# ishine/minimax-speech

Measured on NVIDIA B200. Metric: audio-sec synthesized/sec (24 kHz), higher is better.
Workload: dtype bf16

## Files before the change

minimax-speech_b200/csrc/c_api.cu:

```cuda
#include <atomic>
#include <cstdarg>
#include <mutex>
#include <vector>

#include "dac_enc_engine.h"
#include "dac_engine.h"
#include "engine_common.h"
#include "f32_path.h"
#include "flow_engine.h"
#include "front_engine.h"
#include "profiler.h"
#include "s3_engine.h"

namespace ls {

std::atomic<long long> g_launch_count{0};
long long* g_debug_buffer = nullptr;
bool pdl_enabled() {
  static const bool on = [] {
    const char* e = getenv("LS_NO_PDL");
    return !(e && e[0] == '1');
  }();
  return on;
}
long long g_debug_bytes = 0;
int conv_halo_mode() {
  static const int mode = [] {
    const char* e = getenv("LS_CONV_HALO");
    return e && e[0] >= '0' && e[0] <= '2' ? e[0] - '0' : 2;
  }();
  return mode;
}
bool conv_halo_enabled() { return conv_halo_mode() != 0; }
bool conv_fuse_res_enabled() {
  static const bool on = [] {
    const char* e = getenv("LS_CONV_FUSE_RES");
    return !(e && e[0] == '0');
  }();
  return on;
}
bool conv_dual_enabled() {
  static const bool on = [] {
    const char* e = getenv("LS_CONV_DUAL");
    return !(e && e[0] == '0');
  }();
  return on;
}
bool conv_tma_out_enabled() {
  static const bool on = [] {
    const char* e = getenv("LS_CONV_TMA_OUT");
    return !(e && e[0] == '0');
// ... 666 lines not shown
```

minimax-speech_b200/csrc/conv_gemm.cu:

```cuda
#include <cstdio>
#include <string>
#include <unordered_map>

#include "kernels.h"
#include "profiler.h"
#include "ptx.cuh"

namespace ls {
namespace {

constexpr int kBlockM = 128;
constexpr int kBlockK = 64;
constexpr int kEpiWarps = 16;
constexpr int kEpiThreads = kEpiWarps * 32;
#ifndef CONV_PRODUCER_WARPS
#define CONV_PRODUCER_WARPS 3
#endif
constexpr int kProducerWarps = CONV_PRODUCER_WARPS;
constexpr int kWeightProducers = kProducerWarps - 1;
static_assert(kProducerWarps >= 2, "need one activation and at least one weight producer");
constexpr int kMmaWarp = kProducerWarps;
constexpr int kFirstEpiWarp = kProducerWarps + 1;
constexpr int kThreads = kFirstEpiWarp * 32 + kEpiThreads;
constexpr int kMaxStages = 16;
// ... 234 lines not shown
  fence_proxy_async_smem();
  __syncwarp();
  if (lane == 0) {
    tma_store_3d(map, kF32 ? stg : stg + kOff, n, t_base, b);
    bulk_commit();
  }
}

template <int kKind, int kOff = kStageB16Off>
__device__ __forceinline__ void store_chunk_tma_p(bool one_pending, uint8_t* stg, int lane, const CUtensorMap* map, int n,
                                                  int t_base, int b, bool row_valid, const float (&v)[16]) {
  if (one_pending) store_chunk_tma<kKind, 1, kOff>(stg, lane, map, n, t_base, b, row_valid, v);
  else store_chunk_tma<kKind, 0, kOff>(stg, lane, map, n, t_base, b, row_valid, v);
}

template <int kAct, int kOut0, int kOut1, int kAdd, int kTemb>
__global__ void __launch_bounds__(kThreads, 1)
conv_gemm_kernel(const __grid_constant__ CUtensorMap mapA0, const __grid_constant__ CUtensorMap mapA1,
                 const __grid_constant__ CUtensorMap mapW, const __grid_constant__ CUtensorMap mapOut0,
                 const __grid_constant__ CUtensorMap mapOut1, const __grid_constant__ ConvGemmParams p,
                 const int tmem_cols, const int acc_stride) {
  const int act = kAct >= 0 ? kAct : p.act;
  const int out0_dtype = kOut0 >= 0 ? kOut0 : p.out0_dtype;
  const int out1_mode = kOut1 >= 0 ? kOut1 : p.out1_mode;
  const int add_dtype = kAdd >= 0 ? kAdd : (p.addend_dtype == ADD_GEMM ? (int)ADD_GEMM : p.addend ? p.addend_dtype : (int)OUT_NONE);
  const bool has_temb = kTemb >= 0 ? kTemb != 0 : p.temb != nullptr;
  extern __shared__ uint8_t smem_raw[];
  uint8_t* smem = reinterpret_cast<uint8_t*>((reinterpret_cast<uintptr_t>(smem_raw) + 1023) & ~uintptr_t(1023));
  const int a_bytes = ls_conv_a_stage_bytes(p.a_box_rows);
  const int b_bytes = p.block_n * kBlockK * 2;
  uint8_t* smem_a = smem;
  uint8_t* smem_b = smem + (size_t)p.a_stages * a_bytes;
  uint64_t* bars = reinterpret_cast<uint64_t*>(smem_b + (size_t)p.b_stages * b_bytes);
  uint64_t* a_full = bars;
  uint64_t* a_empty = bars + kMaxStages;
  uint64_t* b_full = bars + 2 * kMaxStages;
  uint64_t* b_empty = bars + 3 * kMaxStages;
  uint64_t* tfull = bars + 4 * kMaxStages;
  uint64_t* tempty = tfull + 2;
  uint32_t* tmem_slot = reinterpret_cast<uint32_t*>(tempty + 2);
  float2* red_base = reinterpret_cast<float2*>(bars + 128);
  uint8_t* stg_base = reinterpret_cast<uint8_t*>(red_base) + p.red_bytes;
  float* svec = reinterpret_cast<float*>(stg_base + kEpiWarps * kStageBytesPerWarp);

  const int warp = threadIdx.x >> 5;
  const int lane = threadIdx.x & 31;
  const int m_tiles = (p.M + kBlockM - 1) / kBlockM;
  const int n_tiles = p.N / p.block_n;
  const int total_tiles = p.B * m_tiles * n_tiles;
  const bool halo = p.halo_mode != 0;
  long long* tl = p.timeline ? p.timeline + (size_t)blockIdx.x * 64 : nullptr;
#define TL(i)                    \
  do {                           \
    if (tl) tl[(i)] = clock64(); \
  } while (0)
// ... 24 lines not shown
      const int tap = r / p.kb_per_tap, kb = r - tap * p.kb_per_tap;
      tma_prefetch_l2_2d(&mapW, kb * kBlockK, tap * p.N + nt * p.block_n);
    }
    for (int j = blockIdx.x; j < p.res_kb; j += gridDim.x) tma_prefetch_l2_2d(&p.res_w, j * kBlockK, 0);
  }
  if (warp == kMmaWarp && lane == 0) {
    for (int i = 0; i < kMaxStages; ++i) {
      mbar_init(&a_full[i], 1);
      mbar_init(&a_empty[i], 1);
      mbar_init(&b_full[i], 1);
      mbar_init(&b_empty[i], (p.dual && !p.b_resident) ? 2 : 1);
    }
    for (int i = 0; i < 2; ++i) {
      mbar_init(&tfull[i], 1);
      mbar_init(&tempty[i], kEpiThreads);
    }
    fence_barrier_init();
  }
  if (warp == 0) {
    __syncwarp();
    tmem_alloc(tmem_slot, (uint32_t)tmem_cols);
    tmem_relinquish();
  }
  {
    auto stage_vec = [&](int off, const float* src, int n) {
      if (off >= 0)
        for (int i = threadIdx.x; i < n; i += kThreads) svec[off + i] = __ldg(src + i);
    };
    stage_vec(p.sv_bias, p.bias, p.chan_mod);
    stage_vec(p.sv_p1a, p.p1_a, p.chan_mod);
    stage_vec(p.sv_p1b, p.p1_b, p.chan_mod);
    stage_vec(p.sv_lng, p.ln_g, p.N);
    stage_vec(p.sv_lnb, p.ln_b, p.N);
  }
  pdl_launch_dependents();
  tc_fence_before();
  __syncthreads();
  tc_fence_after();
  const uint32_t tmem_base = *tmem_slot;
  if (threadIdx.x == 0) TL(1);
  pdl_wait();
  if (threadIdx.x == 0) TL(2);

  auto next_tile = [&](int& cur) -> int {
    while (cur < total_tiles) {
      const int t = cur;
      cur += (int)gridDim.x;
      if (!tile_skipped(p, decode_tile(t, m_tiles, n_tiles))) return t;
    }
    return -1;
  };
  if (p.dual && warp < 2) {
    if (lane == 0) {
      const int depth = p.a_stages >> 1;
      const uint32_t a_tx = (uint32_t)p.a_box_rows * 128u;
      int cur = blockIdx.x, pair = 0, bs = 0;
      uint32_t bph = 0;
      int cnt[2] = {0, 0};
      for (;; ++pair) {
        int t[2];
        t[0] = next_tile(cur);
        if (t[0] < 0) break;
        t[1] = next_tile(cur);
        if (warp == 1 && (!p.b_resident || pair == 0)) {
          for (int kb = 0; kb < p.kb_per_tap; ++kb)
// ... 65 lines not shown
            if (!p.b_resident) {
              umma_commit(&b_empty[bl]);
              if (lone) umma_commit(&b_empty[bl]);
            }
            if (++bl == p.b_stages) bl = 0, bphl ^= 1;
          }
          umma_commit(&a_empty[st]);
        }
        __syncwarp();
        for (int tap = 0; tap < p.taps; ++tap)
          if (++bs == p.b_stages) bs = 0, bph ^= 1;
        ++cnt;
      }
      if (elect_one()) umma_commit(&tfull[m]);
      __syncwarp();
      acc_phase ^= 1;
    }
  } else if (warp < kProducerWarps) {
    if (lane == 0) {
      int as = 0, bs = 0;
      uint32_t aph = 0, bph = 0;
      int b_seq = 0, p_tile = 0;
      int a_seq = 0;
#if CONV_DETAIL_TL == 2
      int dn = 0;
#endif
      const bool a_share = p.b_resident && p.a_stages >= kProducerWarps;
      const uint32_t a_tx = (uint32_t)p.a_box_rows * 128u;
      for (int tile = blockIdx.x; tile < total_tiles; tile += gridDim.x) {
        const TileCoord tc = decode_tile(tile, m_tiles, n_tiles);
// ... 55 lines not shown
            }
            if (++b_seq == kWeightProducers) b_seq = 0;
            if (++bs == p.b_stages) bs = 0, bph ^= 1;
          }
        }
      }
    }
  } else if (warp == kMmaWarp) {
    {
      const uint32_t tmem_u = __shfl_sync(0xffffffffu, tmem_base, 0);
      const uint32_t idesc = make_idesc_bf16(kBlockM, p.block_n, false, false);
      int as = 0, bs = 0;
      uint32_t aph = 0, bph = 0;
      int acc = 0;
      uint32_t acc_phase = 0;
      int n_it = 0, n_tile = 0;
      for (int tile = blockIdx.x; tile < total_tiles; tile += gridDim.x) {
        const TileCoord tc = decode_tile(tile, m_tiles, n_tiles);
        if (__shfl_sync(0xffffffffu, (int)tile_skipped(p, tc), 0)) continue;
        mbar_wait(&tempty[acc], acc_phase ^ 1);
        tc_fence_after();
        const uint32_t d_tmem = tmem_u + (uint32_t)(acc * acc_stride);
        if (halo && p.b_resident && n_tile > 0) {
          for (int kb = 0; kb < p.kb_per_tap; ++kb) {
            mbar_wait(&a_full[as], aph);
            tc_fence_after();
            int nk = kBlockK / 16;
            if (p.k_true > 0 && p.kb_split == p.kb_per_tap) nk = min(nk, (p.k_true - kb * kBlockK + 15) >> 4);
            const uint32_t a_addr = smem_u32(smem_a + (size_t)as * a_bytes);
            const uint32_t b_addr = smem_u32(smem_b) + (uint32_t)(kb * p.taps) * (uint32_t)b_bytes;
// ... 83 lines not shown
#pragma unroll
              for (int k = 0; k < kBlockK / 16; ++k)
                if (k < nk) umma_bf16(d_tmem, adesc + 2 * k, bdesc + 2 * k, idesc, (kb | tap | k) != 0 ? 1u : 0u);
              if (!p.b_resident) umma_commit(&b_empty[bs]);
              if (a_done) umma_commit(&a_empty[as]);
            }
            __syncwarp();
            if (++bs == p.b_stages) bs = 0, bph ^= 1;
            if (a_done) {
              if (++as == p.a_stages) as = 0, aph ^= 1;
            }
          }
        }
        if (elect_one()) umma_commit(&tfull[acc]);
        __syncwarp();
        if (p.res_kb > 0) {
          const uint32_t d2 = tmem_u + (uint32_t)((acc ^ 1) * acc_stride);
          for (int kb2 = 0; kb2 < p.res_kb; ++kb2) {
            mbar_wait(&a_full[as], aph);
            mbar_wait(&b_full[bs], bph);
            tc_fence_after();
            const int nk2 = min(kBlockK / 16, (p.res_k_true - kb2 * kBlockK + 15) >> 4);
            const uint64_t adesc = make_smem_desc_sw128(smem_u32(smem_a + (size_t)as * a_bytes));
            const uint64_t bdesc = make_smem_desc_sw128(smem_u32(smem_b + (size_t)bs * b_bytes));
            if (elect_one()) {
#pragma unroll
              for (int k = 0; k < kBlockK / 16; ++k)
                if (k < nk2) umma_bf16(d2, adesc + 2 * k, bdesc + 2 * k, idesc, (kb2 | k) != 0 ? 1u : 0u);
              umma_commit(&b_empty[bs]);
              umma_commit(&a_empty[as]);
            }
            __syncwarp();
            if (++as == p.a_stages) as = 0, aph ^= 1;
            if (++bs == p.b_stages) bs = 0, bph ^= 1;
          }
          if (elect_one()) umma_commit(&tfull[acc ^ 1]);
          __syncwarp();
        }
        if (tl && lane == 0 && n_it <= p.taps * p.kb_per_tap) tl[32] = clock64();
        if (tl && lane == 0 && n_tile < 8) tl[24 + n_tile] = clock64();
        ++n_tile;
        acc ^= 1;
        if (acc == 0) acc_phase ^= 1;
      }
    }
  } else {
    const int q = warp & 3;
    const int g = (warp - kFirstEpiWarp) >> 2;
    const int row = q * 32 + lane;
    const int n_chunks = p.block_n >> 4;
    uint8_t* stg = stg_base + (warp - kFirstEpiWarp) * kStageBytesPerWarp;
    int acc = 0;
    uint32_t acc_phase = 0;
    uint32_t parity = 0;
    int e_tile = 0;
    for (int tile = blockIdx.x; tile < total_tiles; tile += gridDim.x) {
      const TileCoord tc = decode_tile(tile, m_tiles, n_tiles);
      const int t = tc.mt * kBlockM + row;
      const int n0 = tc.nt * p.block_n;
// ... 57 lines not shown
        const int nxt = tile + (int)gridDim.x;
        if (nxt < total_tiles) {
          const TileCoord nc = decode_tile(nxt, m_tiles, n_tiles);
          const int esz = add_dtype == OUT_F32 ? 4 : 2;
          const int lines = (p.block_n * esz + 127) >> 7;
          const uint8_t* nb = reinterpret_cast<const uint8_t*>(p.addend) + (long long)nc.b * p.out_bstride * esz;
          for (int i = threadIdx.x - kFirstEpiWarp * 32; i < kBlockM * lines; i += kEpiThreads) {
            const int rr = i / lines, ln = i - rr * lines;
            const long long tt = (long long)nc.mt * kBlockM + rr;
            const long long f = tt * p.out_ld + p.out_shift + nc.nt * p.block_n;
            if (tt < p.M && f >= 0 && f + p.block_n <= p.out_alloc)
              asm volatile("prefetch.global.L2 [%0];" ::"l"(nb + f * esz + ln * 128));
          }
        }
      }
      mbar_wait(&tfull[acc], acc_phase);
      tc_fence_after();
      long long* tle = (threadIdx.x == kFirstEpiWarp * 32 && tile == (int)blockIdx.x) ? tl : nullptr;
      if (tle) tle[40] = clock64();
      const uint32_t taddr = tmem_base + ((uint32_t)(q * 32) << 16) + (uint32_t)(acc * acc_stride);
      auto load_x = [&](int c, float (&x)[16]) {
        tmem_ld16(taddr + (uint32_t)(c * 16), reinterpret_cast<uint32_t(&)[16]>(x));
        tmem_ld_wait();
        if (p.bias) {
          const int ch0 = (n0 + c * 16) % p.chan_mod;
          const float4* bp = reinterpret_cast<const float4*>(p.sv_bias >= 0 ? svec + p.sv_bias + ch0 : p.bias + ch0);
#pragma unroll
          for (int g4 = 0; g4 < 4; ++g4) {
            const float4 bv = bp[g4];
            x[4 * g4] += bv.x, x[4 * g4 + 1] += bv.y, x[4 * g4 + 2] += bv.z, x[4 * g4 + 3] += bv.w;
          }
        }
        if (act == ACT_LRELU || act == ACT_LRELU_TANH) {
#pragma unroll
          for (int i = 0; i < 16; ++i) x[i] = x[i] > 0.f ? x[i] : 0.1f * x[i];
// ... 217 lines not shown
  __syncthreads();
  if (threadIdx.x == 0) TL(44);
  if (warp == 0) {
    tc_fence_after();
    tmem_dealloc(tmem_base, (uint32_t)tmem_cols);
  }
#undef TL
}

int pow2_at_least(int x, int lo) {
  int v = lo;
  while (v < x) v <<= 1;
  return v;
}

template <int kAct, int kOut0, int kOut1, int kAdd, int kTemb>
cudaError_t launch_instance(int grid, size_t smem, cudaStream_t stream, const CUtensorMap& mapA0, const CUtensorMap& mapA1,
                            const CUtensorMap& mapW, const CUtensorMap& mapO0, const CUtensorMap& mapO1,
                            const ConvGemmParams& pp, int tmem_cols, int acc_stride) {
  auto* kernel = conv_gemm_kernel<kAct, kOut0, kOut1, kAdd, kTemb>;
  static std::atomic<unsigned long long> optin{0};
  if (cudaError_t e = smem_optin_once(optin, reinterpret_cast<const void*>(kernel), 227 * 1024); e != cudaSuccess) return e;
  return launch_pdl(kernel, dim3(grid), dim3(kThreads), smem, stream, 1, mapA0, mapA1, mapW, mapO0, mapO1, pp, tmem_cols,
                    acc_stride);
}

}

cudaError_t LS_FN(launch_conv_gemm)(const CUtensorMap& mapA0, const CUtensorMap& mapA1, const CUtensorMap& mapW,
                                    const ConvGemmParams& p, int num_sms, cudaStream_t stream) {
#if !LS_HALF_FP16
  if (p.fp16) return launch_conv_gemm_fp16(mapA0, mapA1, mapW, p, num_sms, stream);
#endif
  if (p.block_n % 16 || p.block_n < 16 || p.block_n > 256 || p.N % p.block_n || p.chan_mod % 16) return cudaErrorInvalidValue;
  if ((p.act == ACT_LN_MISH || p.out1_mode == OUT1_LN) && p.block_n != p.N) return cudaErrorInvalidValue;
  if (p.out1_mode == OUT1_LN && p.out0_dtype != OUT_F32) return cudaErrorInvalidValue;
  if (p.out1_mode != OUT1_NONE && p.out1 == nullptr) return cudaErrorInvalidValue;
  if (p.addend_dtype == ADD_GEMM) {
    const long long tiles = (long long)p.B * ((p.M + kBlockM - 1) / kBlockM);
    if (p.res_kb <= 0 || p.res_bias == nullptr || p.N != p.block_n || tiles > num_sms) return cudaErrorInvalidValue;
  } else if (p.res_kb != 0) {
    return cudaErrorInvalidValue;
  }
  ConvGemmParams pp = p;
  pp.timeline = (g_debug_buffer && g_debug_bytes >= 148 * 64 * 8) ? g_debug_buffer : nullptr;
  pp.a_box_rows = p.halo_mode ? conv_halo_box_rows(p.taps, p.dil) : kBlockM;
  if (pp.a_box_rows > 256) return cudaErrorInvalidValue;
  const int a_bytes = ls_conv_a_stage_bytes(pp.a_box_rows);
  const int b_bytes = p.block_n * kBlockK * 2;
  pp.sv_bias = pp.sv_p1a = pp.sv_p1b = pp.sv_lng = pp.sv_lnb = -1;
  pp.sv_floats = 0;
  {
    auto place = [&](int& off, const void* ptr, int n) {
      if (ptr && (pp.sv_floats + n) * 4 <= 16 * 1024) off = pp.sv_floats, pp.sv_floats += (n + 3) & ~3;
    };
    place(pp.sv_bias, p.bias, p.chan_mod);
    if (p.out1_mode == OUT1_SNAKE || p.out1_mode == OUT1_LN) place(pp.sv_p1a, p.p1_a, p.chan_mod), place(pp.sv_p1b, p.p1_b, p.chan_mod);
    if (p.act == ACT_LN_MISH) place(pp.sv_lng, p.ln_g, p.N), place(pp.sv_lnb, p.ln_b, p.N);
  }
  pp.red_bytes = (p.act == ACT_LN_MISH || p.out1_mode == OUT1_LN || p.act < 0) ? kRedBytes : 0;
  const int budget = kSmemBudget + (kRedBytes - pp.red_bytes) - pp.sv_floats * 4;
  const int m_tiles_ = (p.M + kBlockM - 1) / kBlockM;
  const long long tiles_per_cta = ((long long)p.B * m_tiles_ * (p.N / p.block_n) + num_sms - 1) / num_sms;
  const int w_boxes = p.taps * p.kb_per_tap;
  pp.b_resident = 0;
  if (p.N == p.block_n && tiles_per_cta >= 3 && w_boxes <= kMaxStages && w_boxes >= kWeightProducers &&
      w_boxes * b_bytes + 3 * a_bytes <= budget && conv_resident_enabled()) {
    pp.b_resident = 1;
    pp.b_stages = w_boxes;
    pp.a_stages = (budget - w_boxes * b_bytes) / a_bytes;
    if (pp.a_stages > 6) pp.a_stages = 6;
  } else if (p.halo_mode && p.taps > 1) {
    pp.a_stages = p.kb_per_tap > 1 ? 2 : 1;
    if (p.kb_per_tap > 1 && 3 * a_bytes + 4 * b_bytes <= budget) pp.a_stages = CONV_HALO_A_STAGES;
    pp.b_stages = (budget - pp.a_stages * a_bytes) / b_bytes;
  } else {
// ... 6 lines not shown
      if (CONV_DUAL_RESIDENT) {
        pp.dual = 1, pp.b_resident = 1, pp.b_stages = w_boxes;
        pp.a_stages = (budget - w_boxes * b_bytes) / a_bytes;
        if (pp.a_stages > 6) pp.a_stages = 6;
        pp.a_stages &= ~1;
      }
    } else if (4 * a_bytes + 3 * b_bytes <= budget) {
      pp.dual = 1, pp.b_resident = 0, pp.a_stages = 4;
      pp.b_stages = (budget - 4 * a_bytes) / b_bytes;
    }
  }
  if (pp.a_stages > kMaxStages) pp.a_stages = kMaxStages;
  if (pp.b_stages > kMaxStages) pp.b_stages = kMaxStages;
  if (pp.a_stages < 1 || pp.b_stages < 2 || pp.b_stages < kWeightProducers) return cudaErrorInvalidValue;
  const int acc_stride = pow2_at_least(p.block_n, 32);
  const int tmem_cols = 2 * acc_stride;
  size_t smem = (size_t)pp.a_stages * a_bytes + (size_t)pp.b_stages * b_bytes + 1024 + 1024 + pp.red_bytes +
                kEpiWarps * kStageBytesPerWarp + (size_t)pp.sv_floats * 4;
  if (tmem_cols > 256 && smem < 120 * 1024) smem = 120 * 1024;
  const int m_tiles = (p.M + kBlockM - 1) / kBlockM;
  const long long total = (long long)p.B * m_tiles * (p.N / p.block_n);
  if (total <= 0) return cudaSuccess;
  const int grid = (int)(total < num_sms ? total : num_sms);
  const double kt = p.k_true > 0 ? p.k_true : p.kb_per_tap * kBlockK;
  const double rows = (double)p.B * p.M;
  const double out_b = (p.out0_dtype == OUT_F32 ? 4.0 : p.out0_dtype != OUT_NONE ? 2.0 : 0.0) +
                       (p.out1_mode != OUT1_NONE ? 2.0 : 0.0) +
                       (p.addend ? (p.addend_dtype == OUT_F32 ? 4.0 : 2.0) : 0.0);
  ProfScope prof(stream, p.tag == 1 ? PK_CONV_DAC : PK_CONV_FLOW, 2.0 * rows * p.N * (kt * p.taps + (p.res_kb > 0 ? p.res_k_true : 0)),
                 rows * kt * 2.0 + (double)p.taps * p.N * kt * 2.0 + rows * (p.n_store < p.N ? p.n_store : p.N) * out_b);
  count_launch();
  static thread_local std::unordered_map<std::string, CUtensorMap> out_maps;
  auto out_map = [&](const void* base, int elem_bytes, CUtensorMap* dst) -> bool {
    char key[96];
    snprintf(key, sizeof key, "%p/%d/%d/%d/%d", base, elem_bytes, p.N, p.M, p.B);
    auto it = out_maps.find(key);
    if (it == out_maps.end()) {
      CUtensorMap m;
      if (!make_out_map(&m, base, elem_bytes, p.N, p.M, p.B)) return false;
      if (out_maps.size() > 4096) out_maps.clear();
      it = out_maps.emplace(key, m).first;
    }
    *dst = it->second;
    return true;
// ... 13 lines not shown
  const CUtensorMap* mo1 = &mo1v;
  const int add = p.addend_dtype == ADD_GEMM ? (int)ADD_GEMM : p.addend ? p.addend_dtype : (int)OUT_NONE;
  const int temb = p.temb ? 1 : 0;
#define LS_CONV_CASE(A, O0, O1, AD, TE)                                                                          \
  if (p.act == (A) && p.out0_dtype == (O0) && p.out1_mode == (O1) && add == (AD) && temb == (TE))               \
    return launch_instance<A, O0, O1, AD, TE>(grid, smem, stream, mapA0, mapA1, mapW, *mo0, *mo1, pp, tmem_cols, acc_stride);
  LS_CONV_CASE(ACT_LN_MISH, OUT_NONE, OUT1_COPY, OUT_NONE, 1)
  LS_CONV_CASE(ACT_NONE, OUT_F32, OUT1_NONE, OUT_NONE, 0)
  LS_CONV_CASE(ACT_LN_MISH, OUT_F32, OUT1_LN, OUT_F32, 0)
  LS_CONV_CASE(ACT_LN_MISH, OUT_F32, OUT1_NONE, OUT_F32, 0)
  LS_CONV_CASE(ACT_LN_MISH, OUT_F32, OUT1_NONE, ADD_GEMM, 0)
  LS_CONV_CASE(ACT_LN_MISH, OUT_F32, OUT1_LN, ADD_GEMM, 0)
  LS_CONV_CASE(ACT_NONE, OUT_NONE, OUT1_COPY, OUT_NONE, 0)
  LS_CONV_CASE(ACT_LN_MISH, OUT_NONE, OUT1_COPY, OUT_NONE, 0)
#if !LS_HALF_FP16
  LS_CONV_CASE(ACT_LRELU, OUT_NONE, OUT1_COPY, OUT_NONE, 0)
  LS_CONV_CASE(ACT_LRELU, OUT_NONE, OUT1_SNAKE, OUT_NONE, 0)
  LS_CONV_CASE(ACT_NONE, OUT_F32, OUT1_SNAKE, OUT_NONE, 0)
  LS_CONV_CASE(ACT_LRELU, OUT_F32, OUT1_SNAKE, OUT_F32, 0)
  LS_CONV_CASE(ACT_LRELU, OUT_NONE, OUT1_SNAKE, OUT_F32, 0)
  LS_CONV_CASE(ACT_NONE, OUT_F16, OUT1_SNAKE, OUT_NONE, 0)
  LS_CONV_CASE(ACT_LRELU, OUT_F16, OUT1_SNAKE, OUT_F16, 0)
  LS_CONV_CASE(ACT_LRELU, OUT_NONE, OUT1_SNAKE, OUT_F16, 0)
  LS_CONV_CASE(ACT_LRELU_TANH, OUT_F32, OUT1_NONE, OUT_NONE, 0)
#endif
#undef LS_CONV_CASE
  return launch_instance<-1, -1, -1, -1, -1>(grid, smem, stream, mapA0, mapA1, mapW, *mo0, *mo1, pp, tmem_cols, acc_stride);
}

}
// ... 1 lines not shown
```

minimax-speech_b200/csrc/dac_engine.cu:

```cuda
#include <cmath>

#include "dac_engine.h"

namespace ls {

PackedLinear pack_wn_conv(Arena& a, const Weights& w, const std::string& p, int n_pad_to) {
  const ls_tensor& v = w.get(p + ".weight_v");
  const ls_tensor& g = w.get(p + ".weight_g");
  const ls_tensor& b = w.get(p + ".bias");
  require(v.ndim == 3 && g.shape[0] == v.shape[0], "unexpected weight_norm tensors at " + p, LS_ERR_WEIGHTS);
  PackedLinear pl;
  const int N = (int)v.shape[0];
  pl.K = (int)v.shape[1];
  pl.taps = (int)v.shape[2];
  pl.N = n_pad_to > N ? n_pad_to : N;
  pl.block_n = pick_block_n(pl.N);
  pl.w_off = a.reserve((size_t)pl.taps * pl.N * pl.K * 2);
  __nv_bfloat16* dst = reinterpret_cast<__nv_bfloat16*>(a.host(pl.w_off));
  for (size_t i = 0; i < (size_t)pl.taps * pl.N * pl.K; ++i) dst[i] = __float2bfloat16(0.f);
  const size_t per = (size_t)pl.K * pl.taps;
  for (int n = 0; n < N; ++n) {
    double ss = 0;
    for (size_t i = 0; i < per; ++i) ss += (double)v.data[n * per + i] * v.data[n * per + i];
    const float scale = g.data[n] / (float)std::sqrt(ss);
// ... 47 lines not shown

}

struct DacEngine::UnitW {
  PackedLinear conv7, conv1;
  size_t a0, ia0, a2, ia2;
};
struct DacEngine::StageW {
  int stride, cin, cout;
  size_t a_in, ia_in;
  PackedLinear up;
  UnitW unit[3];
};
struct DacEngine::Plan {
  CUtensorMap zt, a0;
  struct {
    CUtensorMap up, d[3];
  } sA[6];
  CUtensorMap sB[6];
};

DacEngine::~DacEngine() {
  if (ws_base_) cudaFree(ws_base_);
}

DacEngine::DacEngine(const Weights& w, int device) : device_(device) {
  LS_CUDA(cudaSetDevice(device));
  cudaDeviceProp prop;
  LS_CUDA(cudaGetDeviceProperties(&prop, device));
  require(prop.major == 10, "this library only runs on sm_100 (B200) devices", LS_ERR_UNSUPPORTED);
  num_sms_ = prop.multiProcessorCount;

  auto snake = [&](const std::string& name, int c, size_t* a_off, size_t* ia_off) {
// ... 93 lines not shown
  const bool halo = conv_halo_enabled();
  auto mk = [&](CUtensorMap* m, size_t off, int C, long long rows, int taps, int dil) {
    require(make_act_map(m, ws_base_ + off, C, (int)rows, B, C, rows * C, halo ? conv_halo_box_rows(taps, dil) : 128),
            "cuTensorMapEncodeTiled failed for an activation buffer", LS_ERR_CUDA);
  };
  static const int dils[3] = {1, 3, 9};
  mk(&pl->zt, o_zt_, latent_, L, 1, 1);
  mk(&pl->a0, o_a0_, latent_, L, 7, 1);
  mk(&pl->sA[0].up, o_sA_[0], dim_, L, 2, 1);
  long long rows = L;
  for (size_t i = 0; i < stages_.size(); ++i) {
    rows *= stages_[i].stride;
    mk(&pl->sA[i + 1].up, o_sA_[(i + 1) & 1], stages_[i].cout, rows, 2, 1);
    for (int j = 0; j < 3; ++j) mk(&pl->sA[i + 1].d[j], o_sA_[(i + 1) & 1], stages_[i].cout, rows, 7, dils[j]);
    mk(&pl->sB[i + 1], o_sB_, stages_[i].cout, rows, 1, 1);
  }
  const Plan& ref = *pl;
  plans_[key] = std::move(pl);
  return ref;
}

void DacEngine::decode(const float* z, const int* lengths, float* wav, int B, int L, cudaStream_t s) {
  require(B > 0 && L > 0, "B and L must be positive");
  require((long long)L * hop_ < (1ll << 31), "utterance too long");
  LS_CUDA(cudaSetDevice(device_));
  ensure_workspace(B, L, s);
  const Plan& pl = plan_for(B, L);
  auto f32 = [&](size_t off) { return arena_.ptr<float>(off); };
  const bool halo = conv_halo_enabled();

  auto conv = [&](const CUtensorMap& a, const PackedLinear& w, long long rows, int rate, int dil, ConvGemmParams p) {
    p.B = B, p.M = (int)rows, p.N = w.N, p.block_n = w.block_n;
    p.taps = w.taps, p.dil = dil, p.pad = (w.taps - 1) / 2 * dil;
    p.kb_per_tap = (w.K + 63) / 64, p.kb_split = p.kb_per_tap;
    p.lengths = lengths, p.m_len_mul = rate, p.m_len_add = 0, p.skip_halo = 64;
    p.bias = w.bias;
    if (p.chan_mod == 0) p.chan_mod = w.N;
    if (p.n_store == 0) p.n_store = w.N;
    if (p.out_ld == 0) {
      p.out_ld = w.N, p.out_shift = 0, p.out_bstride = rows * w.N, p.out_alloc = rows * w.N;
      p.out_valid_mul = (long long)rate * w.N;
    }
    p.k_true = w.K, p.tag = 1, p.halo_mode = halo ? conv_halo_mode() : 0;
    LS_CUDA(launch_conv_gemm(a, a, w.map, p, num_sms_, s));
  };

  LS_CUDA(launch_pack_nct(z, ws<__nv_bfloat16>(o_zt_), B, latent_, L, (long long)latent_ * L, latent_, 0, lengths, s));
  {
    ConvGemmParams p{};
    p.act = ACT_LRELU, p.out1 = ws<void>(o_a0_), p.out1_mode = OUT1_COPY;
    conv(pl.zt, pre_, L, 1, 1, p);
  }
  {
    ConvGemmParams p{};
    p.act = ACT_LRELU, p.out1 = ws<void>(o_sA_[0]), p.out1_mode = OUT1_SNAKE;
    p.p1_a = f32(stages_[0].a_in), p.p1_b = f32(stages_[0].ia_in);
    conv(pl.a0, in_, L, 1, 1, p);
  }
  long long rows = L;
  int rate = 1;
#ifndef LS_DAC_X_F32
#define LS_DAC_X_F32 0
#endif
  constexpr int kXDtype = LS_DAC_X_F32 ? OUT_F32 : OUT_F16;
  void* x = ws<void>(o_x_);
  for (size_t i = 0; i < stages_.size(); ++i) {
    const StageW& st = stages_[i];
    const long long rows_in = rows;
    const int rate_in = rate;
    rows *= st.stride, rate *= st.stride;
    void* sA = ws<void>(o_sA_[(i + 1) & 1]);
    void* sB = ws<void>(o_sB_);
    {
      const int padT = (st.stride + 1) / 2;
      ConvGemmParams p{};
      p.B = B, p.M = (int)rows_in + 1, p.N = st.up.N, p.block_n = st.up.block_n;
      p.taps = 2, p.dil = 1, p.pad = 1;
      p.kb_per_tap = (st.cin + 63) / 64, p.kb_split = p.kb_per_tap;
      p.lengths = lengths, p.m_len_mul = rate_in, p.m_len_add = 1, p.skip_halo = 64;
      p.chan_mod = st.cout, p.bias = st.up.bias, p.act = ACT_NONE;
      p.out0 = x, p.out0_dtype = kXDtype;
      p.out1 = sA, p.out1_mode = OUT1_SNAKE, p.p1_a = f32(st.unit[0].a0), p.p1_b = f32(st.unit[0].ia0);
      p.n_store = st.up.N;
      p.out_ld = st.up.N, p.out_shift = -(long long)padT * st.cout;
      p.out_bstride = rows * st.cout, p.out_alloc = rows * st.cout, p.out_valid_mul = (long long)rate * st.cout;
      p.k_true = st.cin, p.tag = 1, p.halo_mode = halo ? conv_halo_mode() : 0;
      LS_CUDA(launch_conv_gemm(pl.sA[i].up, pl.sA[i].up, st.up.map, p, num_sms_, s));
    }
    static const int dils[3] = {1, 3, 9};
    for (int j = 0; j < 3; ++j) {
      const UnitW& u = st.unit[j];
      {
        ConvGemmParams p{};
        p.act = ACT_LRELU, p.out1 = sB, p.out1_mode = OUT1_SNAKE, p.p1_a = f32(u.a2), p.p1_b = f32(u.ia2);
        conv(pl.sA[i + 1].d[j], u.conv7, rows, rate, dils[j], p);
      }
      {
        ConvGemmParams p{};
        p.act = ACT_LRELU, p.addend = x, p.addend_dtype = kXDtype;
        const bool last_unit = j == 2;
        if (!last_unit) p.out0 = x, p.out0_dtype = kXDtype;
        size_t na, nia;
        if (!last_unit) na = st.unit[j + 1].a0, nia = st.unit[j + 1].ia0;
        else if (i + 1 < stages_.size()) na = stages_[i + 1].a_in, nia = stages_[i + 1].ia_in;
        else na = final_alpha_, nia = final_ialpha_;
        p.out1 = sA, p.out1_mode = OUT1_SNAKE, p.p1_a = f32(na), p.p1_b = f32(nia);
        conv(pl.sB[i + 1], u.conv1, rows, rate, 1, p);
      }
    }
  }
  {
    ConvGemmParams p{};
    p.act = ACT_LRELU_TANH, p.out0 = wav, p.out0_dtype = OUT_F32;
    p.chan_mod = 16, p.n_store = 1, p.zero_skipped = 1;
    p.out_ld = 1, p.out_shift = 0, p.out_bstride = rows, p.out_alloc = rows, p.out_valid_mul = rate;
    conv(pl.sA[stages_.size()].d[0], final_, rows, rate, 1, p);
  }
}

}
```

minimax-speech_b200/csrc/kernels.h:

```cpp
#pragma once
#include <atomic>
#include <cstdint>
#include <cuda.h>
#include <cuda_bf16.h>
#include <cuda_runtime.h>

namespace ls {

extern std::atomic<long long> g_launch_count;
extern long long* g_debug_buffer;
extern long long g_debug_bytes;
inline void count_launch() { g_launch_count.fetch_add(1, std::memory_order_relaxed); }

bool pdl_enabled();
bool conv_halo_enabled();
int conv_halo_mode();
bool conv_fuse_res_enabled();
bool conv_dual_enabled();
bool conv_resident_enabled();
bool conv_tma_out_enabled();
template <typename... KArgs, typename... Args>
inline cudaError_t launch_pdl(void (*kernel)(KArgs...), dim3 grid, dim3 block, size_t smem, cudaStream_t stream,
                              int cluster, Args&&... args) {
  cudaLaunchConfig_t cfg = {};
  cfg.gridDim = grid, cfg.blockDim = block, cfg.dynamicSmemBytes = smem, cfg.stream = stream;
  cudaLaunchAttribute attr[2];
  int n = 0;
  if (cluster > 1) {
    attr[n].id = cudaLaunchAttributeClusterDimension;
    attr[n].val.clusterDim.x = cluster, attr[n].val.clusterDim.y = 1, attr[n].val.clusterDim.z = 1;
    ++n;
  }
// ... 54 lines not shown
  const float* p1_a;
  const float* p1_b;
  int n_store;
  long long out_ld, out_shift, out_bstride, out_alloc, out_valid_mul;
  int k_true, tag;
  int fp16;
  int halo_mode;
  int a_box_rows, a_stages, b_stages;
  int b_resident;
  int tma_out;
  int sv_bias, sv_p1a, sv_p1b, sv_lng, sv_lnb, sv_floats;
  int dual;
  alignas(64) CUtensorMap res_a0, res_a1, res_w;
  int res_kb, res_split, res_k_true;
  const float* res_bias;
  int red_bytes;
  long long* timeline;
};
inline int conv_halo_box_rows(int taps, int dil) { return 128 + (taps - 1) * dil; }
__host__ __device__ constexpr int ls_conv_a_stage_bytes(int box_rows) { return ((box_rows + 7) / 8) * 1024; }

cudaError_t launch_conv_gemm(const CUtensorMap& mapA0, const CUtensorMap& mapA1, const CUtensorMap& mapW,
                             const ConvGemmParams& p, int num_sms, cudaStream_t stream);
cudaError_t launch_conv_gemm_fp16(const CUtensorMap& mapA0, const CUtensorMap& mapA1, const CUtensorMap& mapW,
                                  const ConvGemmParams& p, int num_sms, cudaStream_t stream);

#ifndef ATTN_KV
#define ATTN_KV 64
#endif
struct AttnParams {
// ... 89 lines not shown
```

minimax-speech_b200/csrc/ptx.cuh:

```cuda
#pragma once
#include <cstdint>
#include <cuda.h>
#include <cuda_bf16.h>
#include <cuda_fp16.h>
#include <cuda_runtime.h>

#ifndef LS_HALF_FP16
#define LS_HALF_FP16 0
#endif

namespace ls {

__device__ __forceinline__ uint32_t smem_u32(const void* p) {
  return static_cast<uint32_t>(__cvta_generic_to_shared(p));
}

__device__ __forceinline__ void mbar_init(uint64_t* bar, uint32_t count) {
  asm volatile("mbarrier.init.shared::cta.b64 [%0], %1;" ::"r"(smem_u32(bar)), "r"(count) : "memory");
}
__device__ __forceinline__ void fence_barrier_init() {
  asm volatile("fence.mbarrier_init.release.cluster;" ::: "memory");
}
__device__ __forceinline__ void mbar_arrive_expect_tx(uint64_t* bar, uint32_t bytes) {
  asm volatile("mbarrier.arrive.expect_tx.shared::cta.b64 _, [%0], %1;" ::"r"(smem_u32(bar)), "r"(bytes)
// ... 247 lines not shown
      "tcgen05.st.sync.aligned.32x32b.x32.b32 [%0], "
      "{%1,%2,%3,%4,%5,%6,%7,%8,%9,%10,%11,%12,%13,%14,%15,%16,"
      "%17,%18,%19,%20,%21,%22,%23,%24,%25,%26,%27,%28,%29,%30,%31,%32};"
      ::"r"(taddr), "r"(r[0]), "r"(r[1]), "r"(r[2]), "r"(r[3]), "r"(r[4]), "r"(r[5]), "r"(r[6]), "r"(r[7]),
        "r"(r[8]), "r"(r[9]), "r"(r[10]), "r"(r[11]), "r"(r[12]), "r"(r[13]), "r"(r[14]), "r"(r[15]),
        "r"(r[16]), "r"(r[17]), "r"(r[18]), "r"(r[19]), "r"(r[20]), "r"(r[21]), "r"(r[22]), "r"(r[23]),
        "r"(r[24]), "r"(r[25]), "r"(r[26]), "r"(r[27]), "r"(r[28]), "r"(r[29]), "r"(r[30]), "r"(r[31])
      : "memory");
}
__device__ __forceinline__ void tmem_st16(uint32_t taddr, const uint32_t (&r)[16]) {
  asm volatile(
      "tcgen05.st.sync.aligned.32x32b.x16.b32 [%0], {%1,%2,%3,%4,%5,%6,%7,%8,%9,%10,%11,%12,%13,%14,%15,%16};"
      ::"r"(taddr), "r"(r[0]), "r"(r[1]), "r"(r[2]), "r"(r[3]), "r"(r[4]), "r"(r[5]), "r"(r[6]), "r"(r[7]),
        "r"(r[8]), "r"(r[9]), "r"(r[10]), "r"(r[11]), "r"(r[12]), "r"(r[13]), "r"(r[14]), "r"(r[15])
      : "memory");
}
__device__ __forceinline__ void tmem_st_wait() { asm volatile("tcgen05.wait::st.sync.aligned;" ::: "memory"); }

__device__ __forceinline__ uint64_t make_smem_desc_sw128(uint32_t smem_addr, uint32_t base_offset = 0) {
  uint64_t d = 0;
  d |= static_cast<uint64_t>(base_offset & 7u) << 49;
  d |= static_cast<uint64_t>((smem_addr & 0x3FFFFu) >> 4);
  d |= static_cast<uint64_t>(1) << 16;
  d |= static_cast<uint64_t>(1024 >> 4) << 32;
  d |= static_cast<uint64_t>(1) << 46;
  d |= static_cast<uint64_t>(2) << 61;
  return d;
}

__host__ __device__ constexpr uint32_t make_idesc_bf16(int m, int n, bool a_mn_major, bool b_mn_major,
// ... 121 lines not shown
```

Before: 2390.

## Fuse DAC residual unit dilated conv and 1x1 conv into one chained GEMM kernel

For DAC decoder stages with at most 96 channels, each residual unit's k=7 dilated conv and its following 1x1 conv now run in one kernel launch. The epilogue applies bias, leaky ReLU and snake to the first accumulator in TMEM and writes bf16 back to TMEM. The MMA warp then runs a second tensor-core GEMM against 1x1 weights held resident in shared memory, pipelined one tile behind. This removes a launch and the intermediate activation round trip through global memory, at the cost of doubled TMEM columns, less shared memory for pipeline stages, and an extra epilogue pass.

```diff
diff --git a/minimax-speech_b200/csrc/c_api.cu b/minimax-speech_b200/csrc/c_api.cu
--- a/minimax-speech_b200/csrc/c_api.cu
+++ b/minimax-speech_b200/csrc/c_api.cu
@@ -35,6 +35,13 @@
 bool conv_fuse_res_enabled() {
   static const bool on = [] {
     const char* e = getenv("LS_CONV_FUSE_RES");
+    return !(e && e[0] == '0');
+  }();
+  return on;
+}
+bool dac_fused_ru_enabled() {
+  static const bool on = [] {
+    const char* e = getenv("LS_DAC_FUSED_RU");
     return !(e && e[0] == '0');
   }();
   return on;
diff --git a/minimax-speech_b200/csrc/conv_gemm.cu b/minimax-speech_b200/csrc/conv_gemm.cu
--- a/minimax-speech_b200/csrc/conv_gemm.cu
+++ b/minimax-speech_b200/csrc/conv_gemm.cu
@@ -272,7 +272,7 @@
   else store_chunk_tma<kKind, 0, kOff>(stg, lane, map, n, t_base, b, row_valid, v);
 }
 
-template <int kAct, int kOut0, int kOut1, int kAdd, int kTemb>
+template <int kAct, int kOut0, int kOut1, int kAdd, int kTemb, bool kChain>
 __global__ void __launch_bounds__(kThreads, 1)
 conv_gemm_kernel(const __grid_constant__ CUtensorMap mapA0, const __grid_constant__ CUtensorMap mapA1,
                  const __grid_constant__ CUtensorMap mapW, const __grid_constant__ CUtensorMap mapOut0,
@@ -289,14 +289,19 @@
   const int b_bytes = p.block_n * kBlockK * 2;
   uint8_t* smem_a = smem;
   uint8_t* smem_b = smem + (size_t)p.a_stages * a_bytes;
-  uint64_t* bars = reinterpret_cast<uint64_t*>(smem_b + (size_t)p.b_stages * b_bytes);
+  const int w1_bytes = kChain ? (p.N + kBlockK - 1) / kBlockK * p.N * 128 : 0;
+  uint8_t* smem_w1 = smem_b + (size_t)p.b_stages * b_bytes;
+  uint64_t* bars = reinterpret_cast<uint64_t*>(smem_w1 + w1_bytes);
   uint64_t* a_full = bars;
   uint64_t* a_empty = bars + kMaxStages;
   uint64_t* b_full = bars + 2 * kMaxStages;
   uint64_t* b_empty = bars + 3 * kMaxStages;
   uint64_t* tfull = bars + 4 * kMaxStages;
   uint64_t* tempty = tfull + 2;
-  uint32_t* tmem_slot = reinterpret_cast<uint32_t*>(tempty + 2);
+  uint64_t* hfull = tempty + 2;
+  uint64_t* t1full = hfull + 2;
+  uint64_t* w1full = t1full + 2;
+  uint32_t* tmem_slot = reinterpret_cast<uint32_t*>(w1full + 1);
   float2* red_base = reinterpret_cast<float2*>(bars + 128);
   uint8_t* stg_base = reinterpret_cast<uint8_t*>(red_base) + p.red_bytes;
   float* svec = reinterpret_cast<float*>(stg_base + kEpiWarps * kStageBytesPerWarp);
@@ -351,7 +356,12 @@
     for (int i = 0; i < 2; ++i) {
       mbar_init(&tfull[i], 1);
       mbar_init(&tempty[i], kEpiThreads);
-    }
+      if (kChain) {
+        mbar_init(&hfull[i], kEpiThreads);
+        mbar_init(&t1full[i], 1);
+      }
+    }
+    if (kChain) mbar_init(w1full, 1);
     fence_barrier_init();
   }
   if (warp == 0) {
@@ -369,6 +379,11 @@
     stage_vec(p.sv_p1b, p.p1_b, p.chan_mod);
     stage_vec(p.sv_lng, p.ln_g, p.N);
     stage_vec(p.sv_lnb, p.ln_b, p.N);
+    if (kChain) {
+      stage_vec(p.sv_hb, p.h_bias, p.chan_mod);
+      stage_vec(p.sv_ha, p.h_a, p.chan_mod);
+      stage_vec(p.sv_hia, p.h_ia, p.chan_mod);
+    }
   }
   pdl_launch_dependents();
   tc_fence_before();
@@ -376,6 +391,10 @@
   tc_fence_after();
   const uint32_t tmem_base = *tmem_slot;
   if (threadIdx.x == 0) TL(1);
+  if (kChain && warp == 1 && lane == 0) {
+    mbar_arrive_expect_tx(w1full, (uint32_t)w1_bytes);
+    for (int kb = 0; kb * kBlockK < p.N; ++kb) tma_load_2d(smem_w1 + (size_t)kb * p.N * 128, &p.res_w, w1full, kb * kBlockK, 0);
+  }
   pdl_wait();
   if (threadIdx.x == 0) TL(2);
 
@@ -386,6 +405,24 @@
       if (!tile_skipped(p, decode_tile(t, m_tiles, n_tiles))) return t;
     }
     return -1;
+  };
+  auto chain_mma = [&](uint32_t tmem_u, uint32_t idesc, int s, uint32_t ph) {
+    mbar_wait(w1full, 0);
+    mbar_wait(&hfull[s], ph);
+    tc_fence_after();
+    const uint32_t h = tmem_u + (uint32_t)(s * acc_stride);
+    const uint32_t d1 = tmem_u + (uint32_t)((2 + s) * acc_stride);
+    const uint32_t w1 = smem_u32(smem_w1);
+    const int nj = p.N >> 4;
+    if (elect_one()) {
+#pragma unroll
+      for (int j = 0; j < 8; ++j)
+        if (j < nj)
+          umma_bf16_ts(d1, h + (uint32_t)(16 * j), make_smem_desc_sw128(w1 + (uint32_t)((j >> 2) * p.N * 128)) + 2 * (j & 3),
+                       idesc, j != 0 ? 1u : 0u);
+      umma_commit(&t1full[s]);
+    }
+    __syncwarp();
   };
   if (p.dual && warp < 2) {
     if (lane == 0) {
@@ -481,6 +518,7 @@
       }
       if (elect_one()) umma_commit(&tfull[m]);
       __syncwarp();
+      if (kChain) chain_mma(tmem_u, idesc, m, acc_phase);
       acc_phase ^= 1;
     }
   } else if (warp < kProducerWarps) {
@@ -566,6 +604,8 @@
       uint32_t aph = 0, bph = 0;
       int acc = 0;
       uint32_t acc_phase = 0;
+      int pend = -1;
+      uint32_t pend_ph = 0;
       int n_it = 0, n_tile = 0;
       for (int tile = blockIdx.x; tile < total_tiles; tile += gridDim.x) {
         const TileCoord tc = decode_tile(tile, m_tiles, n_tiles);
@@ -679,6 +719,10 @@
         }
         if (elect_one()) umma_commit(&tfull[acc]);
         __syncwarp();
+        if (kChain) {
+          if (pend >= 0) chain_mma(tmem_u, idesc, pend, pend_ph);
+          pend = acc, pend_ph = acc_phase;
+        }
         if (p.res_kb > 0) {
           const uint32_t d2 = tmem_u + (uint32_t)((acc ^ 1) * acc_stride);
           for (int kb2 = 0; kb2 < p.res_kb; ++kb2) {
@@ -708,6 +752,7 @@
         acc ^= 1;
         if (acc == 0) acc_phase ^= 1;
       }
+      if (kChain && pend >= 0) chain_mma(tmem_u, idesc, pend, pend_ph);
     }
   } else {
     const int q = warp & 3;
@@ -795,11 +840,48 @@
           }
         }
       }
-      mbar_wait(&tfull[acc], acc_phase);
+      if (kChain) {
+        mbar_wait(&tfull[acc], acc_phase);
+        tc_fence_after();
+        const uint32_t hrow = tmem_base + ((uint32_t)(q * 32) << 16) + (uint32_t)(acc * acc_stride);
+#pragma unroll 1
+        for (int c = g; c < n_chunks; c += 4) {
+          float x[16];
+          tmem_ld16(hrow + (uint32_t)(c * 16), reinterpret_cast<uint32_t(&)[16]>(x));
+          tmem_ld_wait();
+          const int ch0 = (n0 + c * 16) % p.chan_mod;
+          const float4* bp = reinterpret_cast<const float4*>(p.sv_hb >= 0 ? svec + p.sv_hb + ch0 : p.h_bias + ch0);
+          const float4* ap = reinterpret_cast<const float4*>(p.sv_ha >= 0 ? svec + p.sv_ha + ch0 : p.h_a + ch0);
+          const float4* ip = reinterpret_cast<const float4*>(p.sv_hia >= 0 ? svec + p.sv_hia + ch0 : p.h_ia + ch0);
+#pragma unroll
+          for (int g4 = 0; g4 < 4; ++g4) {
+            const float4 bv = bp[g4];
+            x[4 * g4] += bv.x, x[4 * g4 + 1] += bv.y, x[4 * g4 + 2] += bv.z, x[4 * g4 + 3] += bv.w;
+          }
+#pragma unroll
+          for (int i = 0; i < 16; ++i) x[i] = x[i] > 0.f ? x[i] : 0.1f * x[i];
+#pragma unroll
+          for (int g4 = 0; g4 < 4; ++g4) {
+            const float4 al = ap[g4], ia = ip[g4];
+            x[4 * g4 + 0] = snake_f(x[4 * g4 + 0], al.x, ia.x);
+            x[4 * g4 + 1] = snake_f(x[4 * g4 + 1], al.y, ia.y);
+            x[4 * g4 + 2] = snake_f(x[4 * g4 + 2], al.z, ia.z);
+            x[4 * g4 + 3] = snake_f(x[4 * g4 + 3], al.w, ia.w);
+          }
+          uint32_t pk[8];
+#pragma unroll
+          for (int k = 0; k < 8; ++k) pk[k] = row_valid ? LS_PACK_H2(x[2 * k], x[2 * k + 1]) : 0u;
+          tmem_st8(hrow + (uint32_t)(c * 16), pk);
+        }
+        tmem_st_wait();
+        tc_fence_before();
+        mbar_arrive(&hfull[acc]);
+      }
+      mbar_wait(kChain ? &t1full[acc] : &tfull[acc], acc_phase);
       tc_fence_after();
       long long* tle = (threadIdx.x == kFirstEpiWarp * 32 && tile == (int)blockIdx.x) ? tl : nullptr;
       if (tle) tle[40] = clock64();
-      const uint32_t taddr = tmem_base + ((uint32_t)(q * 32) << 16) + (uint32_t)(acc * acc_stride);
+      const uint32_t taddr = tmem_base + ((uint32_t)(q * 32) << 16) + (uint32_t)((kChain ? 2 + acc : acc) * acc_stride);
       auto load_x = [&](int c, float (&x)[16]) {
         tmem_ld16(taddr + (uint32_t)(c * 16), reinterpret_cast<uint32_t(&)[16]>(x));
         tmem_ld_wait();
@@ -1047,11 +1129,11 @@
   return v;
 }
 
-template <int kAct, int kOut0, int kOut1, int kAdd, int kTemb>
+template <int kAct, int kOut0, int kOut1, int kAdd, int kTemb, bool kChain = false>
 cudaError_t launch_instance(int grid, size_t smem, cudaStream_t stream, const CUtensorMap& mapA0, const CUtensorMap& mapA1,
                             const CUtensorMap& mapW, const CUtensorMap& mapO0, const CUtensorMap& mapO1,
                             const ConvGemmParams& pp, int tmem_cols, int acc_stride) {
-  auto* kernel = conv_gemm_kernel<kAct, kOut0, kOut1, kAdd, kTemb>;
+  auto* kernel = conv_gemm_kernel<kAct, kOut0, kOut1, kAdd, kTemb, kChain>;
   static std::atomic<unsigned long long> optin{0};
   if (cudaError_t e = smem_optin_once(optin, reinterpret_cast<const void*>(kernel), 227 * 1024); e != cudaSuccess) return e;
   return launch_pdl(kernel, dim3(grid), dim3(kThreads), smem, stream, 1, mapA0, mapA1, mapW, mapO0, mapO1, pp, tmem_cols,
@@ -1075,6 +1157,9 @@
   } else if (p.res_kb != 0) {
     return cudaErrorInvalidValue;
   }
+  if (p.chain && (!p.halo_mode || p.taps < 2 || p.N != p.block_n || p.N > 128 || p.act != ACT_LRELU || p.addend_dtype == ADD_GEMM ||
+                  !p.h_bias || !p.h_a || !p.h_ia || LS_HALF_FP16))
+    return cudaErrorInvalidValue;
   ConvGemmParams pp = p;
   pp.timeline = (g_debug_buffer && g_debug_bytes >= 148 * 64 * 8) ? g_debug_buffer : nullptr;
   pp.a_box_rows = p.halo_mode ? conv_halo_box_rows(p.taps, p.dil) : kBlockM;
@@ -1090,9 +1175,12 @@
     place(pp.sv_bias, p.bias, p.chan_mod);
     if (p.out1_mode == OUT1_SNAKE || p.out1_mode == OUT1_LN) place(pp.sv_p1a, p.p1_a, p.chan_mod), place(pp.sv_p1b, p.p1_b, p.chan_mod);
     if (p.act == ACT_LN_MISH) place(pp.sv_lng, p.ln_g, p.N), place(pp.sv_lnb, p.ln_b, p.N);
+    pp.sv_hb = pp.sv_ha = pp.sv_hia = -1;
+    if (p.chain) place(pp.sv_hb, p.h_bias, p.chan_mod), place(pp.sv_ha, p.h_a, p.chan_mod), place(pp.sv_hia, p.h_ia, p.chan_mod);
   }
   pp.red_bytes = (p.act == ACT_LN_MISH || p.out1_mode == OUT1_LN || p.act < 0) ? kRedBytes : 0;
-  const int budget = kSmemBudget + (kRedBytes - pp.red_bytes) - pp.sv_floats * 4;
+  const int w1_bytes = p.chain ? (p.N + kBlockK - 1) / kBlockK * p.N * 128 : 0;
+  const int budget = kSmemBudget + (kRedBytes - pp.red_bytes) - pp.sv_floats * 4 - w1_bytes;
   const int m_tiles_ = (p.M + kBlockM - 1) / kBlockM;
   const long long tiles_per_cta = ((long long)p.B * m_tiles_ * (p.N / p.block_n) + num_sms - 1) / num_sms;
   const int w_boxes = p.taps * p.kb_per_tap;
@@ -1129,8 +1217,8 @@
   if (pp.b_stages > kMaxStages) pp.b_stages = kMaxStages;
   if (pp.a_stages < 1 || pp.b_stages < 2 || pp.b_stages < kWeightProducers) return cudaErrorInvalidValue;
   const int acc_stride = pow2_at_least(p.block_n, 32);
-  const int tmem_cols = 2 * acc_stride;
-  size_t smem = (size_t)pp.a_stages * a_bytes + (size_t)pp.b_stages * b_bytes + 1024 + 1024 + pp.red_bytes +
+  const int tmem_cols = (p.chain ? 4 : 2) * acc_stride;
+  size_t smem = (size_t)pp.a_stages * a_bytes + (size_t)pp.b_stages * b_bytes + w1_bytes + 1024 + 1024 + pp.red_bytes +
                 kEpiWarps * kStageBytesPerWarp + (size_t)pp.sv_floats * 4;
   if (tmem_cols > 256 && smem < 120 * 1024) smem = 120 * 1024;
   const int m_tiles = (p.M + kBlockM - 1) / kBlockM;
@@ -1142,7 +1230,8 @@
   const double out_b = (p.out0_dtype == OUT_F32 ? 4.0 : p.out0_dtype != OUT_NONE ? 2.0 : 0.0) +
                        (p.out1_mode != OUT1_NONE ? 2.0 : 0.0) +
                        (p.addend ? (p.addend_dtype == OUT_F32 ? 4.0 : 2.0) : 0.0);
-  ProfScope prof(stream, p.tag == 1 ? PK_CONV_DAC : PK_CONV_FLOW, 2.0 * rows * p.N * (kt * p.taps + (p.res_kb > 0 ? p.res_k_true : 0)),
+  ProfScope prof(stream, p.tag == 1 ? PK_CONV_DAC : PK_CONV_FLOW,
+                 2.0 * rows * p.N * (kt * p.taps + (p.res_kb > 0 ? p.res_k_true : 0) + (p.chain ? p.N : 0)),
                  rows * kt * 2.0 + (double)p.taps * p.N * kt * 2.0 + rows * (p.n_store < p.N ? p.n_store : p.N) * out_b);
   count_launch();
   static thread_local std::unordered_map<std::string, CUtensorMap> out_maps;
@@ -1186,6 +1275,15 @@
   LS_CONV_CASE(ACT_NONE, OUT_NONE, OUT1_COPY, OUT_NONE, 0)
   LS_CONV_CASE(ACT_LN_MISH, OUT_NONE, OUT1_COPY, OUT_NONE, 0)
 #if !LS_HALF_FP16
+  if (p.chain) {
+    if (p.out0_dtype == OUT_F16 && p.out1_mode == OUT1_SNAKE && add == OUT_F16 && temb == 0)
+      return launch_instance<ACT_LRELU, OUT_F16, OUT1_SNAKE, OUT_F16, 0, true>(grid, smem, stream, mapA0, mapA1, mapW, *mo0, *mo1, pp,
+                                                                             tmem_cols, acc_stride);
+    if (p.out0_dtype == OUT_NONE && p.out1_mode == OUT1_SNAKE && add == OUT_F16 && temb == 0)
+      return launch_instance<ACT_LRELU, OUT_NONE, OUT1_SNAKE, OUT_F16, 0, true>(grid, smem, stream, mapA0, mapA1, mapW, *mo0, *mo1, pp,
+                                                                              tmem_cols, acc_stride);
+    return cudaErrorInvalidValue;
+  }
   LS_CONV_CASE(ACT_LRELU, OUT_NONE, OUT1_COPY, OUT_NONE, 0)
   LS_CONV_CASE(ACT_LRELU, OUT_NONE, OUT1_SNAKE, OUT_NONE, 0)
   LS_CONV_CASE(ACT_NONE, OUT_F32, OUT1_SNAKE, OUT_NONE, 0)
diff --git a/minimax-speech_b200/csrc/dac_engine.cu b/minimax-speech_b200/csrc/dac_engine.cu
--- a/minimax-speech_b200/csrc/dac_engine.cu
+++ b/minimax-speech_b200/csrc/dac_engine.cu
@@ -85,9 +85,9 @@
 };
 struct DacEngine::Plan {
   CUtensorMap zt, a0;
-  struct {
+  struct Views {
     CUtensorMap up, d[3];
-  } sA[6];
+  } sA[6], sBh[6];
   CUtensorMap sB[6];
 };
 
@@ -211,6 +211,8 @@
     mk(&pl->sA[i + 1].up, o_sA_[(i + 1) & 1], stages_[i].cout, rows, 2, 1);
     for (int j = 0; j < 3; ++j) mk(&pl->sA[i + 1].d[j], o_sA_[(i + 1) & 1], stages_[i].cout, rows, 7, dils[j]);
     mk(&pl->sB[i + 1], o_sB_, stages_[i].cout, rows, 1, 1);
+    mk(&pl->sBh[i + 1].up, o_sB_, stages_[i].cout, rows, 2, 1);
+    for (int j = 0; j < 3; ++j) mk(&pl->sBh[i + 1].d[j], o_sB_, stages_[i].cout, rows, 7, dils[j]);
   }
   const Plan& ref = *pl;
   plans_[key] = std::move(pl);
@@ -231,7 +233,7 @@
     p.taps = w.taps, p.dil = dil, p.pad = (w.taps - 1) / 2 * dil;
     p.kb_per_tap = (w.K + 63) / 64, p.kb_split = p.kb_per_tap;
     p.lengths = lengths, p.m_len_mul = rate, p.m_len_add = 0, p.skip_halo = 64;
-    p.bias = w.bias;
+    if (p.bias == nullptr) p.bias = w.bias;
     if (p.chan_mod == 0) p.chan_mod = w.N;
     if (p.n_store == 0) p.n_store = w.N;
     if (p.out_ld == 0) {
@@ -261,6 +263,7 @@
 #endif
   constexpr int kXDtype = LS_DAC_X_F32 ? OUT_F32 : OUT_F16;
   void* x = ws<void>(o_x_);
+  const Plan::Views* in_views = &pl.sA[0];
   for (size_t i = 0; i < stages_.size(); ++i) {
     const StageW& st = stages_[i];
     const long long rows_in = rows;
@@ -282,11 +285,26 @@
       p.out_ld = st.up.N, p.out_shift = -(long long)padT * st.cout;
       p.out_bstride = rows * st.cout, p.out_alloc = rows * st.cout, p.out_valid_mul = (long long)rate * st.cout;
       p.k_true = st.cin, p.tag = 1, p.halo_mode = halo ? conv_halo_mode() : 0;
-      LS_CUDA(launch_conv_gemm(pl.sA[i].up, pl.sA[i].up, st.up.map, p, num_sms_, s));
+      LS_CUDA(launch_conv_gemm(in_views->up, in_views->up, st.up.map, p, num_sms_, s));
     }
     static const int dils[3] = {1, 3, 9};
+    const bool fused = dac_fused_ru_enabled() && halo && kXDtype == OUT_F16 && st.cout <= 96 && st.unit[0].conv1.N == st.cout;
     for (int j = 0; j < 3; ++j) {
       const UnitW& u = st.unit[j];
+      const bool last_unit = j == 2;
+      size_t na, nia;
+      if (!last_unit) na = st.unit[j + 1].a0, nia = st.unit[j + 1].ia0;
+      else if (i + 1 < stages_.size()) na = stages_[i + 1].a_in, nia = stages_[i + 1].ia_in;
+      else na = final_alpha_, nia = final_ialpha_;
+      if (fused) {
+        ConvGemmParams p{};
+        p.chain = 1, p.h_bias = u.conv7.bias, p.h_a = f32(u.a2), p.h_ia = f32(u.ia2), p.res_w = u.conv1.map;
+        p.act = ACT_LRELU, p.bias = u.conv1.bias, p.addend = x, p.addend_dtype = kXDtype;
+        if (!last_unit) p.out0 = x, p.out0_dtype = kXDtype;
+        p.out1 = j % 2 ? sA : sB, p.out1_mode = OUT1_SNAKE, p.p1_a = f32(na), p.p1_b = f32(nia);
+        conv(j % 2 ? pl.sBh[i + 1].d[j] : pl.sA[i + 1].d[j], u.conv7, rows, rate, dils[j], p);
+        continue;
+      }
       {
         ConvGemmParams p{};
         p.act = ACT_LRELU, p.out1 = sB, p.out1_mode = OUT1_SNAKE, p.p1_a = f32(u.a2), p.p1_b = f32(u.ia2);
@@ -295,24 +313,20 @@
       {
         ConvGemmParams p{};
         p.act = ACT_LRELU, p.addend = x, p.addend_dtype = kXDtype;
-        const bool last_unit = j == 2;
         if (!last_unit) p.out0 = x, p.out0_dtype = kXDtype;
-        size_t na, nia;
-        if (!last_unit) na = st.unit[j + 1].a0, nia = st.unit[j + 1].ia0;
-        else if (i + 1 < stages_.size()) na = stages_[i + 1].a_in, nia = stages_[i + 1].ia_in;
-        else na = final_alpha_, nia = final_ialpha_;
         p.out1 = sA, p.out1_mode = OUT1_SNAKE, p.p1_a = f32(na), p.p1_b = f32(nia);
         conv(pl.sB[i + 1], u.conv1, rows, rate, 1, p);
       }
     }
+    in_views = fused ? &pl.sBh[i + 1] : &pl.sA[i + 1];
   }
   {
     ConvGemmParams p{};
     p.act = ACT_LRELU_TANH, p.out0 = wav, p.out0_dtype = OUT_F32;
     p.chan_mod = 16, p.n_store = 1, p.zero_skipped = 1;
     p.out_ld = 1, p.out_shift = 0, p.out_bstride = rows, p.out_alloc = rows, p.out_valid_mul = rate;
-    conv(pl.sA[stages_.size()].d[0], final_, rows, rate, 1, p);
-  }
-}
-
-}
+    conv(in_views->d[0], final_, rows, rate, 1, p);
+  }
+}
+
+}
diff --git a/minimax-speech_b200/csrc/kernels.h b/minimax-speech_b200/csrc/kernels.h
--- a/minimax-speech_b200/csrc/kernels.h
+++ b/minimax-speech_b200/csrc/kernels.h
@@ -16,6 +16,7 @@
 bool conv_halo_enabled();
 int conv_halo_mode();
 bool conv_fuse_res_enabled();
+bool dac_fused_ru_enabled();
 bool conv_dual_enabled();
 bool conv_resident_enabled();
 bool conv_tma_out_enabled();
@@ -100,6 +101,11 @@
   alignas(64) CUtensorMap res_a0, res_a1, res_w;
   int res_kb, res_split, res_k_true;
   const float* res_bias;
+  int chain;
+  const float* h_bias;
+  const float* h_a;
+  const float* h_ia;
+  int sv_hb, sv_ha, sv_hia;
   int red_bytes;
   long long* timeline;
 };
diff --git a/minimax-speech_b200/csrc/ptx.cuh b/minimax-speech_b200/csrc/ptx.cuh
--- a/minimax-speech_b200/csrc/ptx.cuh
+++ b/minimax-speech_b200/csrc/ptx.cuh
@@ -285,6 +285,11 @@
       ::"r"(taddr), "r"(r[0]), "r"(r[1]), "r"(r[2]), "r"(r[3]), "r"(r[4]), "r"(r[5]), "r"(r[6]), "r"(r[7]),
         "r"(r[8]), "r"(r[9]), "r"(r[10]), "r"(r[11]), "r"(r[12]), "r"(r[13]), "r"(r[14]), "r"(r[15])
       : "memory");
+}
+__device__ __forceinline__ void tmem_st8(uint32_t taddr, const uint32_t (&r)[8]) {
+  asm volatile("tcgen05.st.sync.aligned.32x32b.x8.b32 [%0], {%1,%2,%3,%4,%5,%6,%7,%8};" ::"r"(taddr), "r"(r[0]), "r"(r[1]),
+               "r"(r[2]), "r"(r[3]), "r"(r[4]), "r"(r[5]), "r"(r[6]), "r"(r[7])
+               : "memory");
 }
 __device__ __forceinline__ void tmem_st_wait() { asm volatile("tcgen05.wait::st.sync.aligned;" ::: "memory"); }
 
diff --git a/profiles/dac_launches.py b/profiles/dac_launches.py
--- /dev/null
+++ b/profiles/dac_launches.py
@@ -0,0 +1,43 @@
+import os
+import sys
+
+sys.path.insert(0, os.path.dirname(os.path.dirname(os.path.abspath(__file__))))
+import torch
+from torch.profiler import ProfilerActivity, profile
+
+import minimax_speech_b200.synth as synth
+from minimax_speech_b200.dac import DACVAEDecoder
+
+B = int(sys.argv[1]) if len(sys.argv) > 1 else 16
+L = int(sys.argv[2]) if len(sys.argv) > 2 else 500
+fused = os.environ.get("LS_DAC_FUSED_RU", "1") != "0"
+dev = torch.device("cuda:0")
+dac = DACVAEDecoder()
+dac.load_state_dict(synth.dac_decoder_state_dict(0, "reference"))
+z = torch.cat([synth.dac_latents(b, L) for b in range(B)], 0).to(dev)
+for _ in range(3):
+    dac.decode(z)
+torch.cuda.synchronize()
+reps = 5
+with profile(activities=[ProfilerActivity.CUDA]) as prof:
+    for _ in range(reps):
+        dac.decode(z)
+    torch.cuda.synchronize()
+ev = sorted((e for e in prof.events() if e.device_type == torch.autograd.DeviceType.CUDA and "conv_gemm" in e.name),
+            key=lambda e: e.time_range.start)
+per = len(ev) // reps
+assert per * reps == len(ev), "unexpected launch count"
+us = [min(ev[r * per + i].time_range.elapsed_us() for r in range(reps)) for i in range(per)]
+chans = [768, 384, 192, 96, 48]
+i, rows = 2, []
+print(f"LS_DAC_FUSED_RU={int(fused)}  decode {B} x {L} frames, conv_gemm launches, min of {reps} (us)")
+print(f"  pre + input conv: {us[0]:.0f} + {us[1]:.0f}")
+total_ru = 0.0
+for s, c in enumerate(chans):
+    one = fused and c <= 96
+    n = 3 if one else 6
+    ru = us[i + 1:i + 1 + n]
+    print(f"  stage {s + 1} C={c:4d}: up {us[i]:6.0f}  RU launches " + " / ".join(f"{v:.0f}" for v in ru) + f"  RU sum {sum(ru):7.0f}")
+    total_ru += sum(ru)
+    i += 1 + n
+print(f"  final conv: {us[i]:.0f}   all conv_gemm: {sum(us):.0f} us, ResidualUnits {total_ru:.0f} us")
```

After: 2405 (median of 6 runs). About the same (+0.6%).
